# yashsoni501/PQP-for-MPC

Measured on AMD Instinct MI355X. Metric: PQP iterations/sec (and QP-instances/sec) at fixed n_dual, higher is better.
Workload: dtype f32; 1 GPU; BASELINE configs[3] (N=1) / configs[4] (N=8): synthetic n_dual=1024, M=512, 4096 independent problems per GPU, fixed-iteration updateY2; n_dual=1024, batch_per_gpu=4096, global_batch=4096, iters_per_launch=10, parallelism=problem-sharded x1 (no data-path collective)

## Files before the change

### pqp-for-mpc_amd/csrc/pqp_halfsched.h

```cpp
#pragma once

#if defined(__HIPCC__) || defined(__CUDACC__)
#define PQP_HS_HD __host__ __device__ inline
#else
#define PQP_HS_HD inline
#endif

namespace pqp {
namespace hs {

constexpr int kWaves = 16;
constexpr int kTile = 64;
constexpr int kTileStride = 65;
constexpr int kTileWords = kTile * kTileStride;
constexpr int kSlots = 9;
constexpr int kHalfCols = 32;

PQP_HS_HD int steps(int C) { return C > 0 ? kWaves * C + kWaves - 1 : 0; }

PQP_HS_HD int partner(int T, int wave) { return (((T - wave) % kWaves) + kWaves) % kWaves; }

PQP_HS_HD bool active(int T, int wave, int C) {
    const int s = T - wave;
    return s >= 0 && s < kWaves * C;
}
PQP_HS_HD int update_of(int T, int wave) { return (T - wave) / kWaves; }
PQP_HS_HD int kblock_of(int T, int wave) { return (T - wave) % kWaves; }


PQP_HS_HD int tile_rows(int T, int wave) {
    const int p = partner(T, wave);
    return wave < p ? wave : p;
}
PQP_HS_HD int tile_cols(int T, int wave) {
    const int p = partner(T, wave);
    return wave < p ? p : wave;
}
PQP_HS_HD bool transposed(int T, int wave) { return wave > partner(T, wave); }
PQP_HS_HD bool diagonal(int T, int wave) { return partner(T, wave) == wave; }

PQP_HS_HD int load_halves(int T, int wave, int C) {
    if (!active(T, wave, C)) return 0;
    const int p = partner(T, wave);
    return p == wave ? 3 : (wave < p ? 1 : 2);
}

PQP_HS_HD int first_half_col(int halves) { return (halves & 1) ? 0 : kHalfCols; }

PQP_HS_HD int slot(int T, int wave) {
    const int t = ((T % kWaves) + kWaves) % kWaves;
    const int p = partner(T, wave);
    const int lo = wave < p ? wave : p;
    return (wave + p == t) ? lo : lo - (t + 1) / 2;
}

PQP_HS_HD int y_read_buf(int h) { return h & 1; }
PQP_HS_HD int y_write_buf(int h) { return (h + 1) & 1; }

PQP_HS_HD bool last_kblock(int T, int wave) { return kblock_of(T, wave) == kWaves - 1; }

constexpr int kFlagWords = 2 * kSlots + 2 * kWaves;
PQP_HS_HD int tile_flag(int T, int wave, int half) { return 2 * slot(T, wave) + half; }
PQP_HS_HD int y_flag(int buf, int kblock) { return 2 * kSlots + buf * kWaves + kblock; }
PQP_HS_HD int half_of(int halves) { return halves >> 1; }
PQP_HS_HD bool y_dirty(unsigned bits) { return !(bits < 0x7f800000u); }
PQP_HS_HD float q_fold(float s, float q) { return __builtin_fmaf(q, 0.0f, s); }
PQP_HS_HD bool q_dirty(float s) { return s != s; }

}
}
```

### pqp-for-mpc_amd/csrc/pqp_kernels.hip

```cpp
#include <atomic>
#include <type_traits>

#include "pqp_device.h"
#include "pqp_halfsched.h"
#include "pqp_launch.h"

namespace pqp {

static inline unsigned cdiv(long long a, long long b) { return (unsigned)((a + b - 1) / b); }
static bool aligned16(const void* p);

__device__ __forceinline__ float4 ld4(const float* p) { return *reinterpret_cast<const float4*>(p); }
typedef float f32x4 __attribute__((ext_vector_type(4)));
template <bool NTL>
__device__ __forceinline__ float4 ldq4(const float* p) {
    if constexpr (NTL) {
        const f32x4 v = __builtin_nontemporal_load(reinterpret_cast<const f32x4*>(p));
        return make_float4(v.x, v.y, v.z, v.w);
    } else {
        return *reinterpret_cast<const float4*>(p);
    }
}

struct Acc4 {
// ... 50 lines not shown
}

template <bool NTL>
__device__ __forceinline__ void literal_segment(Acc4& a, const float* __restrict__ col, int ldq, int ka, int kb,
                                                const float* __restrict__ y, int row, const float th[4]) {
    int k = ka;
    const float* src = col + (size_t)k * ldq;
    for (; k + 4 <= kb; k += 4) {
        float4 q[4];
#pragma unroll
        for (int j = 0; j < 4; ++j) q[j] = ldq4<NTL>(src + (size_t)j * ldq);
        src += (size_t)4 * ldq;
        const float4 y0 = *reinterpret_cast<const float4*>(y + k);
        literal4(a, q[0], y0.x, k + 0, row, th);
        literal4(a, q[1], y0.y, k + 1, row, th);
        literal4(a, q[2], y0.z, k + 2, row, th);
        literal4(a, q[3], y0.w, k + 3, row, th);
    }
    for (; k < kb; ++k) {
        literal4(a, ldq4<NTL>(src), y[k], k, row, th);
        src += ldq;
    }
}

template <int U, bool NTL, typename OutPtr>
__device__ __forceinline__ void update_rows4(const float* __restrict__ Q, int ldq, int N, int row, int w0,
                                             const float* __restrict__ th_g, const float* __restrict__ fd_g,
                                             const float* __restrict__ y, OutPtr out) {
    Acc4 a;
#pragma unroll
    for (int r = 0; r < 4; ++r) a.p[r] = a.n[r] = 0.0f;
    float th[4];
#pragma unroll
    for (int r = 0; r < 4; ++r) th[r] = (row + r < N) ? th_g[row + r] : 0.0f;
    const float* col = Q + row;
    const int wa = w0 < N ? w0 : N;
    const int wb = (w0 + 256) < N ? (w0 + 256) : N;
    lean_segment<U, NTL>(a, col, ldq, 0, wa, y);
    literal_segment<NTL>(a, col, ldq, wa, wb, y, row, th);
    lean_segment<U, NTL>(a, col, ldq, wb, N, y);
#pragma unroll
    for (int r = 0; r < 4; ++r) {
        const int i = row + r;
        if (i < N) {
            const float f = fd_g[i];
            const float num = a.n[r] + 1.0f * max_ref(0.0f, -f);
            const float den = a.p[r] + 1.0f * max_ref(0.0f, f);
            out[i] = num / den * y[i];
        }
    }
}

template <int NT, int U = 8, bool NTL = false>
__global__ void __launch_bounds__(NT) k_batch_iterate(const float* __restrict__ QdT, long long qstride, int ldq,
                                                      int N, const float* __restrict__ theta,
                                                      const float* __restrict__ Fd, int ldv,
                                                      const float* Y0, float* Y, int updates) {
    extern __shared__ __attribute__((aligned(16))) float lds[];
    float* ya = lds;
    float* yb = lds + ldq;
    const int b = blockIdx.x;
    const int tid = threadIdx.x;
    const float* Q = QdT + (size_t)b * (size_t)qstride;
    const float* th = theta + (size_t)b * ldv;
    const float* fd = Fd + (size_t)b * ldv;
    for (int i = tid; i < ldq; i += NT) {
        ya[i] = (i < N) ? (Y0 ? Y0[(size_t)b * ldv + i] : 1000.0f) : 0.0f;
        yb[i] = 0.0f;
    }
    __syncthreads();
    const int wave = tid >> 6;
    for (int u = 0; u < updates; ++u) {
        float* cur = (u & 1) ? yb : ya;
        float* nxt = (u & 1) ? ya : yb;
        for (int r0 = 0; r0 < N; r0 += 4 * NT) {
            const int row = r0 + 4 * tid;
            const int w0 = r0 + 256 * wave;
            if (row < N) update_rows4<U, NTL, float*>(Q, ldq, N, row, w0, th, fd, cur, nxt);
        }
        __syncthreads();
    }
    const float* fin = (updates & 1) ? yb : ya;
    for (int i = tid; i < N; i += NT) Y[(size_t)b * ldv + i] = fin[i];
}

template <int U, bool NTL>
__device__ __forceinline__ void stream_load(float4 (&q)[U], const float* __restrict__ src, int ldq) {
#pragma unroll
    for (int j = 0; j < U; ++j) q[j] = ldq4<NTL>(src + (size_t)j * ldq);
}
template <int U>
__device__ __forceinline__ void stream_block(Acc4& a, const float4 (&q)[U], int k0, bool literal,
                                             const float* __restrict__ y, int row, const float th[4]) {
    if (literal) {
#pragma unroll
        for (int j = 0; j < U; j += 4) {
            const float4 yv = *reinterpret_cast<const float4*>(y + k0 + j);
            literal4(a, q[j + 0], yv.x, k0 + j + 0, row, th);
            literal4(a, q[j + 1], yv.y, k0 + j + 1, row, th);
            literal4(a, q[j + 2], yv.z, k0 + j + 2, row, th);
            literal4(a, q[j + 3], yv.w, k0 + j + 3, row, th);
        }
    } else {
#pragma unroll
        for (int j = 0; j < U; j += 4) {
            const float4 yv = *reinterpret_cast<const float4*>(y + k0 + j);
            lean4(a, q[j + 0], yv.x);
            lean4(a, q[j + 1], yv.y);
            lean4(a, q[j + 2], yv.z);
            lean4(a, q[j + 3], yv.w);
        }
    }
}
template <int U, bool NTL>
__global__ void __launch_bounds__(256) k_batch_stream(const float* __restrict__ QdT, long long qstride, int ldq,
                                                      int N, const float* __restrict__ theta,
                                                      const float* __restrict__ Fd, int ldv,
                                                      const float* Y0, float* Y, int updates) {
    extern __shared__ __attribute__((aligned(16))) float lds[];
    float* ya = lds;
    float* yb = lds + ldq;
    const int b = blockIdx.x;
    const int tid = threadIdx.x, wave = tid >> 6;
    const float* Q = QdT + (size_t)b * (size_t)qstride;
    const float* th_g = theta + (size_t)b * ldv;
    const float* fd_g = Fd + (size_t)b * ldv;
    for (int i = tid; i < ldq; i += 256) {
        ya[i] = (i < N) ? (Y0 ? Y0[(size_t)b * ldv + i] : 1000.0f) : 0.0f;
        yb[i] = 0.0f;
    }
    const int nb = N / U, npass = N / 1024;
    float4 qa[U], qb[U];
    if (updates > 0) stream_load<U, NTL>(qa, Q + 4 * tid, ldq);
    __syncthreads();
    for (int u = 0; u < updates; ++u) {
        const float* cur = (u & 1) ? yb : ya;
        float* nxt = (u & 1) ? ya : yb;
        for (int pass = 0; pass < npass; ++pass) {
            const int row = pass * 1024 + 4 * tid;
            const int wa = pass * 1024 + 256 * wave, wbd = wa + 256;
            Acc4 a;
#pragma unroll
            for (int r = 0; r < 4; ++r) a.p[r] = a.n[r] = 0.0f;
            float th[4];
#pragma unroll
            for (int r = 0; r < 4; ++r) th[r] = th_g[row + r];
            const float* col = Q + row;
            for (int kb = 0; kb < nb; kb += 2) {
                stream_load<U, NTL>(qb, col + (size_t)(kb + 1) * U * ldq, ldq);
                int k0 = kb * U;
                stream_block<U>(a, qa, k0, k0 >= wa && k0 < wbd, cur, row, th);
                if (kb + 2 < nb) stream_load<U, NTL>(qa, col + (size_t)(kb + 2) * U * ldq, ldq);
                else if (pass + 1 < npass) stream_load<U, NTL>(qa, Q + (pass + 1) * 1024 + 4 * tid, ldq);
                else if (u + 1 < updates) stream_load<U, NTL>(qa, Q + 4 * tid, ldq);
                k0 += U;
                stream_block<U>(a, qb, k0, k0 >= wa && k0 < wbd, cur, row, th);
            }
#pragma unroll
            for (int r = 0; r < 4; ++r) {
                const int i = row + r;
                const float f = fd_g[i];
                const float num = a.n[r] + 1.0f * max_ref(0.0f, -f);
                const float den = a.p[r] + 1.0f * max_ref(0.0f, f);
                nxt[i] = num / den * cur[i];
            }
        }
        __syncthreads();
    }
    const float* fin = (updates & 1) ? yb : ya;
    for (int i = tid; i < N; i += 256) Y[(size_t)b * ldv + i] = fin[i];
}

template <int U, int RL, int RA = 0>
__global__ void __launch_bounds__(256) k_batch_resident(const float* __restrict__ QdT, long long qstride, int ldq,
                                                        const float* __restrict__ theta,
                                                        const float* __restrict__ Fd, int ldv, const float* Y0,
                                                        float* Y, int updates) {
    constexpr int N = 1024, nb = N / U, P = RA + RL;
    static_assert((nb - P) % 2 == 0, "the streamed blocks come in pairs");
    extern __shared__ __attribute__((aligned(16))) float lds[];
    float* ya = lds;
    float* yb = lds + ldq;
    float4* res = reinterpret_cast<float4*>(lds + 2 * ldq);
    const int b = blockIdx.x;
    const int tid = threadIdx.x, wave = tid >> 6;
    const float* Q = QdT + (size_t)b * (size_t)qstride;
    const float* th_g = theta + (size_t)b * ldv;
    const float* fd_g = Fd + (size_t)b * ldv;
    for (int i = tid; i < ldq; i += 256) {
        ya[i] = (i < N) ? (Y0 ? Y0[(size_t)b * ldv + i] : 1000.0f) : 0.0f;
        yb[i] = 0.0f;
    }
    const int row = 4 * tid;
    const int wa = 256 * wave, wbd = wa + 256;
    const float* col = Q + row;
    float th[4];
#pragma unroll
    for (int r = 0; r < 4; ++r) th[r] = th_g[row + r];
    const unsigned long long qaddr = (unsigned long long)Q;
    const __amdgpu_buffer_rsrc_t rs = __builtin_amdgcn_make_buffer_rsrc(
        (void*)(((unsigned long long)__builtin_amdgcn_readfirstlane((unsigned)(qaddr >> 32)) << 32) |
                (unsigned)__builtin_amdgcn_readfirstlane((unsigned)qaddr)),
        (short)0, __builtin_amdgcn_readfirstlane((int)(qstride * 4)), 0x00020000);
    auto ld = [&](float4(&q)[U], int kb, bool nt) {
        if constexpr (RA > 0) {
            const int s0 = kb * U * ldq * 4;
            if (nt) {
#pragma unroll
                for (int j = 0; j < U; ++j) {
                    const f32x4 v = __builtin_amdgcn_raw_buffer_load_b128(rs, 16 * tid, s0 + j * ldq * 4, 2);
                    q[j] = make_float4(v.x, v.y, v.z, v.w);
                }
            } else {
#pragma unroll
                for (int j = 0; j < U; ++j) {
                    const f32x4 v = __builtin_amdgcn_raw_buffer_load_b128(rs, 16 * tid, s0 + j * ldq * 4, 0);
                    q[j] = make_float4(v.x, v.y, v.z, v.w);
                }
            }
        } else {
            if (nt) stream_load<U, true>(q, col + (size_t)kb * U * ldq, ldq);
            else stream_load<U, false>(q, col + (size_t)kb * U * ldq, ldq);
        }
    };
    float4 qa[U], qb[U];
    float4 rr[RA > 0 ? RA * U : 1];
    if (updates > 0) {
#pragma unroll
        for (int rb = 0; rb < RA; ++rb) {
            float4 t[U];
            ld(t, rb, true);
#pragma unroll
            for (int j = 0; j < U; ++j) rr[rb * U + j] = t[j];
        }
        ld(qa, P, false);
    }
    __syncthreads();
    for (int u = 0; u < updates; ++u) {
        const float* cur = (u & 1) ? yb : ya;
        float* nxt = (u & 1) ? ya : yb;
#pragma unroll
        for (int j = 0; j < RA * U; ++j) {
            asm volatile("" : "+a"(rr[j].x));
            asm volatile("" : "+a"(rr[j].y));
            asm volatile("" : "+a"(rr[j].z));
            asm volatile("" : "+a"(rr[j].w));
        }
        Acc4 a;
#pragma unroll
        for (int r = 0; r < 4; ++r) a.p[r] = a.n[r] = 0.0f;
#pragma unroll
        for (int rb = 0; rb < RA; ++rb) {
            float4 q[U];
#pragma unroll
            for (int j = 0; j < U; ++j) q[j] = rr[rb * U + j];
            const int k0 = rb * U;
            stream_block<U>(a, q, k0, k0 >= wa && k0 < wbd, cur, row, th);
        }
#pragma unroll
        for (int lb = 0; lb < RL; ++lb) {
            float4* slot = res + (size_t)lb * U * 256 + tid;
            if (u == 0) {
                ld(qb, RA + lb, true);
#pragma unroll
                for (int j = 0; j < U; ++j) slot[j * 256] = qb[j];
            } else {
#pragma unroll
                for (int j = 0; j < U; ++j) qb[j] = slot[j * 256];
            }
            const int k0 = (RA + lb) * U;
            stream_block<U>(a, qb, k0, k0 >= wa && k0 < wbd, cur, row, th);
        }
        for (int kb = P; kb < nb; kb += 2) {
            ld(qb, kb + 1, true);
            int k0 = kb * U;
            stream_block<U>(a, qa, k0, k0 >= wa && k0 < wbd, cur, row, th);
            if (kb + 2 < nb)
                ld(qa, kb + 2, true);
            else if (u + 1 < updates)
                ld(qa, P, false);
            k0 += U;
            stream_block<U>(a, qb, k0, k0 >= wa && k0 < wbd, cur, row, th);
        }
#pragma unroll
        for (int r = 0; r < 4; ++r) {
            const int i = row + r;
            const float f = fd_g[i];
            const float num = a.n[r] + 1.0f * max_ref(0.0f, -f);
            const float den = a.p[r] + 1.0f * max_ref(0.0f, f);
            nxt[i] = num / den * cur[i];
        }
        __syncthreads();
    }
    const float* fin = (updates & 1) ? yb : ya;
    for (int i = tid; i < N; i += 256) Y[(size_t)b * ldv + i] = fin[i];
}

__device__ __forceinline__ void lean1(float& ap, float& an, float q, float y) {
    const float z = 0.0f * y;
    const float p = q * y;
    ap += (q < 0.0f) ? z : p;
    an += (q > 0.0f) ? z : -p;
}
template <int SK, bool DIAG>
__device__ __forceinline__ void half_tile_sum(float& ap, float& an, const float* __restrict__ q,
                                              const float* __restrict__ yk, int lane, float th) {
    constexpr int CH = 8;
#pragma unroll 1
    for (int c = 0; c < hs::kTile; c += CH) {
        float qv[CH];
#pragma unroll
        for (int j = 0; j < CH; ++j) qv[j] = q[(c + j) * SK];
#pragma unroll
        for (int j = 0; j < CH; j += 4) {
            const float4 yv = *reinterpret_cast<const float4*>(yk + c + j);
            if constexpr (DIAG) {
                literal1(ap, an, qv[j + 0], yv.x, (c + j + 0 == lane) ? th : 0.0f);
                literal1(ap, an, qv[j + 1], yv.y, (c + j + 1 == lane) ? th : 0.0f);
                literal1(ap, an, qv[j + 2], yv.z, (c + j + 2 == lane) ? th : 0.0f);
                literal1(ap, an, qv[j + 3], yv.w, (c + j + 3 == lane) ? th : 0.0f);
            } else {
                lean1(ap, an, qv[j + 0], yv.x);
                lean1(ap, an, qv[j + 1], yv.y);
                lean1(ap, an, qv[j + 2], yv.z);
                lean1(ap, an, qv[j + 3], yv.w);
            }
        }
    }
}
typedef float hf2 __attribute__((ext_vector_type(2)));
template <int SK>
__device__ __forceinline__ void half_tile_sum_pf(float& ap, float& an, const float* __restrict__ q,
                                                 const float* __restrict__ yk) {
    constexpr int CH = 16;
    hf2 acc = {ap, an};
#pragma unroll 1
    for (int c = 0; c < hs::kTile; c += CH) {
        float qv[CH];
#pragma unroll
        for (int j = 0; j < CH; ++j) qv[j] = q[(c + j) * SK];
#pragma unroll
        for (int j = 0; j < CH; j += 4) {
            const float4 yv = *reinterpret_cast<const float4*>(yk + c + j);
            const hf2 p01 = hf2{qv[j + 0], qv[j + 1]} * hf2{yv.x, yv.y};
            const hf2 p23 = hf2{qv[j + 2], qv[j + 3]} * hf2{yv.z, yv.w};
#pragma unroll
            for (int h = 0; h < 4; ++h) {
                const float p = h < 2 ? p01[h] : p23[h - 2];
                float tp, tn;
                asm("v_max_f32 %0, %1, 0" : "=v"(tp) : "v"(p));
                asm("v_max_f32_e64 %0, -%1, 0" : "=v"(tn) : "v"(p));
                acc += hf2{tp, tn};
            }
        }
    }
    ap = acc.x;
    an = acc.y;
}
__device__ __forceinline__ int half_y_flag(float y) {
    return __builtin_amdgcn_ballot_w64(hs::y_dirty(__float_as_uint(y))) != 0;
}
__device__ __forceinline__ float half_q_fold(float s, f32x4 q) {
    return hs::q_fold(hs::q_fold(hs::q_fold(hs::q_fold(s, q.x), q.y), q.z), q.w);
}
constexpr size_t kHalfLdsBytes =
    ((size_t)2 * 1024 + (size_t)hs::kSlots * hs::kTileWords + hs::kFlagWords) * sizeof(float);
static_assert(kHalfLdsBytes <= 160 * 1024, "k_batch_half: LDS of a gfx950 CU");
template <bool PF>
__global__ void __launch_bounds__(1024) k_batch_half(const float* __restrict__ QdT, long long qstride, int ldq,
                                                     const float* __restrict__ theta, const float* __restrict__ Fd,
                                                     int ldv, const float* Y0, float* Y, int updates) {
    constexpr int N = 1024;
    constexpr int HL = hs::kHalfCols / 4;
    extern __shared__ __attribute__((aligned(16))) float lds[];
    float* ybuf = lds;
    float* tiles = lds + 2 * N;
    int* flags = reinterpret_cast<int*>(tiles + hs::kSlots * hs::kTileWords);
    const int b = blockIdx.x;
    const int tid = threadIdx.x, lane = tid & 63;
    const int wave = __builtin_amdgcn_readfirstlane(tid >> 6);
    const float* Q = QdT + (size_t)b * (size_t)qstride;
    const int row = hs::kTile * wave + lane;
    const float ys = Y0 ? Y0[(size_t)b * ldv + tid] : 1000.0f;
    ybuf[tid] = ys;
    ybuf[N + tid] = 0.0f;
    if constexpr (PF) {
        flags[hs::y_flag(0, wave)] = half_y_flag(ys);
        flags[hs::y_flag(1, wave)] = 1;
    }
    const float th = theta[(size_t)b * ldv + row];
    const float f = Fd[(size_t)b * ldv + row];
    const int lk = lane >> 4, lr = 4 * (lane & 15);
    f32x4 pa[HL], pb[HL];
    auto issue = [&](int T) {
        const int halves = hs::load_halves(T, wave, updates);
        if (halves == 0) return;
        const int k0 = hs::kTile * hs::tile_cols(T, wave) + hs::first_half_col(halves) + lk;
        const float* src = Q + (size_t)k0 * ldq + hs::kTile * hs::tile_rows(T, wave) + lr;
#pragma unroll
        for (int j = 0; j < HL; ++j)
            pa[j] = __builtin_nontemporal_load(reinterpret_cast<const f32x4*>(src + (size_t)(4 * j) * ldq));
        if (halves == 3) {
#pragma unroll
            for (int j = 0; j < HL; ++j)
                pb[j] = __builtin_nontemporal_load(
                    reinterpret_cast<const f32x4*>(src + (size_t)(hs::kHalfCols + 4 * j) * ldq));
        }
    };
    auto stash = [&](int T) {
        const int halves = hs::load_halves(T, wave, updates);
        if (halves == 0) return;
        float* dst = tiles + hs::slot(T, wave) * hs::kTileWords + (hs::first_half_col(halves) + lk) * hs::kTileStride + lr;
        float fold = 0.0f;
#pragma unroll
        for (int j = 0; j < HL; ++j) {
            float* d = dst + 4 * j * hs::kTileStride;
            d[0] = pa[j].x, d[1] = pa[j].y, d[2] = pa[j].z, d[3] = pa[j].w;
            if constexpr (PF) fold = half_q_fold(fold, pa[j]);
        }
        if constexpr (PF) {
            if (halves != 3)
                flags[hs::tile_flag(T, wave, hs::half_of(halves))] =
                    __builtin_amdgcn_ballot_w64(hs::q_dirty(fold)) != 0;
        }
        if (halves == 3) {
#pragma unroll
            for (int j = 0; j < HL; ++j) {
                float* d = dst + (hs::kHalfCols + 4 * j) * hs::kTileStride;
                d[0] = pb[j].x, d[1] = pb[j].y, d[2] = pb[j].z, d[3] = pb[j].w;
            }
        }
    };
    const int S = hs::steps(updates);
    issue(0);
    __syncthreads();
    if (updates == 0) Y[(size_t)b * ldv + tid] = ybuf[tid];
    float ap = 0.0f, an = 0.0f;
    for (int T = 0; T < S; ++T) {
        stash(T);
        __syncthreads();
        issue(T + 1);
        if (hs::active(T, wave, updates)) {
            const int h = hs::update_of(T, wave), K = hs::kblock_of(T, wave);
            const float* cur = ybuf + hs::y_read_buf(h) * N;
            const float* yk = cur + hs::kTile * K;
            const float* tile = tiles + hs::slot(T, wave) * hs::kTileWords;
            if (K == 0) ap = an = 0.0f;
            if (hs::diagonal(T, wave))
                half_tile_sum<hs::kTileStride, true>(ap, an, tile + lane, yk, lane, th);
            else {
                bool fast = false;
                if constexpr (PF) {
                    const int dirty = flags[hs::tile_flag(T, wave, 0)] | flags[hs::tile_flag(T, wave, 1)] |
                                      flags[hs::y_flag(hs::y_read_buf(h), K)];
                    fast = __builtin_amdgcn_readfirstlane(dirty) == 0;
                }
                if (hs::transposed(T, wave)) {
                    if (fast) half_tile_sum_pf<1>(ap, an, tile + lane * hs::kTileStride, yk);
                    else half_tile_sum<1, false>(ap, an, tile + lane * hs::kTileStride, yk, lane, th);
                } else {
                    if (fast) half_tile_sum_pf<hs::kTileStride>(ap, an, tile + lane, yk);
                    else half_tile_sum<hs::kTileStride, false>(ap, an, tile + lane, yk, lane, th);
                }
            }
            if (hs::last_kblock(T, wave)) {
                const float num = an + 1.0f * max_ref(0.0f, -f);
                const float den = ap + 1.0f * max_ref(0.0f, f);
                const float yn = num / den * cur[row];
                ybuf[hs::y_write_buf(h) * N + row] = yn;
                if constexpr (PF)
                    flags[hs::y_flag(hs::y_write_buf(h), wave)] = half_y_flag(yn);
                if (h == updates - 1) Y[(size_t)b * ldv + row] = yn;
            }
        }
        __syncthreads();
    }
}

template <int NT, int U = 8, bool NTL = false>
__global__ void __launch_bounds__(NT) k_batch_update(const float* __restrict__ QdT, long long qstride, int ldq,
                                                     int N, const float* __restrict__ theta,
                                                     const float* __restrict__ Fd, int ldv,
                                                     const float* __restrict__ Yin, float* __restrict__ Yout) {
    extern __shared__ __attribute__((aligned(16))) float lds[];
    const int b = blockIdx.y;
    const int tid = threadIdx.x;
    const float* yg = Yin + (size_t)b * ldv;
    for (int i = tid; i < ldq; i += NT) lds[i] = (i < N) ? yg[i] : 0.0f;
    __syncthreads();
    const int r0 = blockIdx.x * 4 * NT;
    const int row = r0 + 4 * tid;
    const int w0 = r0 + 256 * (tid >> 6);
    if (row < N)
        update_rows4<U, NTL>(QdT + (size_t)b * (size_t)qstride, ldq, N, row, w0, theta + (size_t)b * ldv,
                     Fd + (size_t)b * ldv, lds, Yout + (size_t)b * ldv);
}

__global__ void __launch_bounds__(256) k_update_split(const float* __restrict__ QpT, const float* __restrict__ QnT,
                                                      int ldq, int N, const float* __restrict__ Fdp,
                                                      const float* __restrict__ Fdn, const float* __restrict__ Y,
                                                      float* __restrict__ Ynext) {
    const int i = blockIdx.x * 256 + threadIdx.x;
    if (i >= N) return;
    float num = 0.0f, den = 0.0f;
    for (int k = 0; k < N; ++k) num += QnT[(size_t)k * ldq + i] * Y[k];
    for (int k = 0; k < N; ++k) den += QpT[(size_t)k * ldq + i] * Y[k];
    num = num + 1.0f * Fdn[i];
    den = den + 1.0f * Fdp[i];
    Ynext[i] = num / den * Y[i];
}

__host__ __device__ inline int split_wgs(int rows, int lw) { return (2 * rows + lw - 1) / lw; }

__global__ void __launch_bounds__(256) k_build_split(const float* __restrict__ Qd, int ld,
                                                     const float* __restrict__ theta, const float* __restrict__ Fd,
                                                     int N, int rows, int row0, int lw, float* __restrict__ SP,
                                                     float* __restrict__ fdpn) {
    const int KB = split_kblocks(N);
    const long long e = (long long)blockIdx.x * 256 + threadIdx.x;
    if (e < (long long)rows * 4 * KB) {
        const int i = (int)(e / (4 * KB)), k = (int)(e % (4 * KB));
        float qn = 0.0f, qp = 0.0f;
        if (k < N) {
            const float q = Qd[(size_t)i * ld + k];
            const float t = (row0 + i == k) ? theta[i] : 0.0f;
            qn = max_ref(0.0f, -q) + 1.0f * t;
            qp = max_ref(0.0f, q) + 1.0f * t;
        }
        const int p = 2 * i;
        const size_t base = (((size_t)(p / lw) * KB + (k >> 2)) * lw + (p % lw)) * 4 + (k & 3);
        SP[base] = qn;
        SP[base + 4] = qp;
    }
    if (e < rows) {
        const float fd = Fd[row0 + e];
        fdpn[2 * e + 0] = max_ref(0.0f, -fd);
        fdpn[2 * e + 1] = max_ref(0.0f, fd);
    }
}

__global__ void __launch_bounds__(256) k_theta_rows(const float* __restrict__ Qd, int ld, int N, int rows,
                                                    float* __restrict__ theta) {
    const int i = blockIdx.x * 256 + threadIdx.x;
    if (i >= rows) return;
    float s = 0.0f;
    for (int k = 0; k < N; ++k) s += max_ref(0.0f, -Qd[(size_t)i * ld + k]) * 1.0f;
    theta[i] = max_ref(s, 5.0f);
}

__device__ inline void stage_y_lds(const float* __restrict__ Y, int N, int n_lds, float* ys) {
    const int t = threadIdx.x;
    int done = 0;
    if ((reinterpret_cast<uintptr_t>(Y) & 15) == 0) {
        const int N4 = N >> 2;
        const float4* Y4 = reinterpret_cast<const float4*>(Y);
        for (int b = 0; b < N4; b += 64 * 8) {
            float4 v[8];
#pragma unroll
            for (int j = 0; j < 8; ++j) {
                const int i = b + 64 * j + t;
                v[j] = (i < N4) ? Y4[i] : make_float4(0.0f, 0.0f, 0.0f, 0.0f);
            }
#pragma unroll
            for (int j = 0; j < 8; ++j) {
                const int i = b + 64 * j + t;
                if (i < N4) reinterpret_cast<float4*>(ys)[i] = v[j];
            }
        }
        done = 4 * N4;
    }
    for (int b = done; b < n_lds; b += 64 * 16) {
        float v[16];
#pragma unroll
        for (int j = 0; j < 16; ++j) {
            const int k = b + 64 * j + t;
            v[j] = (k < N) ? Y[k] : 0.0f;
        }
#pragma unroll
        for (int j = 0; j < 16; ++j) {
            const int k = b + 64 * j + t;
            if (k < n_lds) ys[k] = v[j];
        }
    }
    __syncthreads();
}

template <int W, int S>
__global__ void __launch_bounds__(64 * W) k_split_relay(const float* __restrict__ SP, const float* __restrict__ fdpn,
                                                        int N, int rows, int row0, int lw,
                                                        const float* __restrict__ Yin, float* __restrict__ Yout,
                                                        const int* __restrict__ gate, int* __restrict__ err,
                                                        int spin_max) {
    if (gate && *gate != kStatusContinue) return;
    extern __shared__ __attribute__((aligned(16))) float lds[];
    unsigned long long* slot = reinterpret_cast<unsigned long long*>(lds);
    float* ys = lds + 128;
    const int KB = split_kblocks(N);
    const int lane = threadIdx.x & 63, w = __builtin_amdgcn_readfirstlane(threadIdx.x >> 6);
    const int ll = lane % lw;
    const int p = blockIdx.x * lw + ll;
    const bool live = lane < lw && p < 2 * rows;
    const int G = (KB + S - 1) / S;
    typedef float f4v __attribute__((ext_vector_type(4)));
    typedef float f2v __attribute__((ext_vector_type(2)));
    const float* region = SP + (size_t)blockIdx.x * KB * lw * 4;
    const __amdgpu_buffer_rsrc_t rs =
        __builtin_amdgcn_make_buffer_rsrc(const_cast<float*>(region), (short)0, KB * lw * 16, 0x00020000);
    const int vo = ll * 16, kstride = lw * 16;
    f4v q[S];
    const bool lane_loads = lane < lw;
    auto load_seg = [&](int g) {
        const int nj = KB - g * S;
#pragma unroll
        for (int j = 0; j < S; ++j)
            q[j] = (j < nj && lane_loads) ? __builtin_amdgcn_raw_buffer_load_b128(rs, vo, (g * S + j) * kstride, 0)
                                          : f4v{0.0f, 0.0f, 0.0f, 0.0f};
    };
    if (w < G) load_seg(w);
    const float fd = live ? fdpn[p] : 0.0f;
    {
        const int t = threadIdx.x, n_lds = 4 * G * S;
        for (int b = 0; b < n_lds; b += 64 * W * 8) {
            float v[8];
#pragma unroll
            for (int j = 0; j < 8; ++j) {
                const int k = b + 64 * W * j + t;
                v[j] = (k < N) ? Yin[k] : 0.0f;
            }
#pragma unroll
            for (int j = 0; j < 8; ++j) {
                const int k = b + 64 * W * j + t;
                if (k < n_lds) ys[k] = v[j];
            }
        }
        if (w == 0) slot[lane] = 0ull;
    }
    __syncthreads();
    float acc = 0.0f;
    bool stale = false;
    for (int g = w; g < G; g += W) {
#pragma unroll
        for (int j0 = 0; j0 < S; j0 += 4) {
            f4v y[4];
#pragma unroll
            for (int u = 0; u < 4; ++u) y[u] = *reinterpret_cast<const f4v*>(ys + 4 * (g * S + j0 + u));
#pragma unroll
            for (int u = 0; u < 4; ++u) {
                const int j = j0 + u;
                const f2v lo = f2v{q[j].x, q[j].y} * f2v{y[u].x, y[u].y};
                const f2v hi = f2v{q[j].z, q[j].w} * f2v{y[u].z, y[u].w};
                q[j] = f4v{lo.x, lo.y, hi.x, hi.y};
            }
#pragma unroll
            for (int u = 0; u < 4; ++u) asm volatile("" : "+v"(q[j0 + u]));
        }
        const unsigned long long h = relay_wait(slot, lane, g, spin_max, stale);
        __builtin_amdgcn_s_setprio(3);
        acc = __uint_as_float((unsigned)h);
#pragma unroll
        for (int j = 0; j < S; ++j) {
            acc += q[j].x;
            acc += q[j].y;
            acc += q[j].z;
            acc += q[j].w;
        }
        __hip_atomic_store(slot + lane, ((unsigned long long)(g + 1) << 32) | __float_as_uint(acc), __ATOMIC_RELAXED,
                           __HIP_MEMORY_SCOPE_WORKGROUP);
        __builtin_amdgcn_s_setprio(0);
        if (g + W < G) load_seg(g + W);
    }
    if (w == (G - 1) % W) {
        const float v = acc + 1.0f * fd;
        const float den = __shfl_xor(v, 1);
        if (!(p & 1) && live) {
            const int i = p >> 1;
            Yout[i] = v / den * ys[row0 + i];
        }
    }
    relay_report(stale, err, lane);
}

constexpr int kLeanS = 16;
__global__ void __launch_bounds__(256) k_build_lean(const float* __restrict__ Qd, int ld,
                                                    const float* __restrict__ theta, const float* __restrict__ Fd,
                                                    int N, int rows, int row0, int lw, float* __restrict__ LP,
                                                    float* __restrict__ aux) {
    const int KB = split_kblocks(N);
    const int rp = lw >> 1;
    const long long e = (long long)blockIdx.x * 256 + threadIdx.x;
    if (e < (long long)rows * 4 * KB) {
        const int i = (int)(e / (4 * KB)), k = (int)(e % (4 * KB));
        const size_t at = (((size_t)(i / rp) * KB + (k >> 2)) * rp + (i % rp)) * 4 + (k & 3);
        const float q = k < N ? Qd[(size_t)i * ld + k] : 0.0f;
        LP[at] = q;
        if (q != q) {
            const int G = (KB + kLeanS - 1) / kLeanS, nwg = (rows + rp - 1) / rp;
            int* segnan = reinterpret_cast<int*>(aux + 4 * (size_t)nwg * rp);
            atomicOr(segnan + (size_t)(i / rp) * G + (k >> 2) / kLeanS, 1);
        }
    }
    if (e < rows) {
        const float fd = Fd[row0 + e];
        aux[4 * e + 0] = max_ref(0.0f, -fd);
        aux[4 * e + 1] = max_ref(0.0f, fd);
        aux[4 * e + 2] = theta[e];
        aux[4 * e + 3] = 0.0f;
    }
}

template <int W, int S>
__global__ void __launch_bounds__(64 * W) k_lean_relay(const float* __restrict__ LP, const float* __restrict__ aux,
                                                       int N, int rows, int row0, int lw,
                                                       const float* __restrict__ Yin, float* __restrict__ Yout,
                                                       const int* __restrict__ gate, int* __restrict__ err,
                                                       int spin_max) {
    if (gate && *gate != kStatusContinue) return;
    extern __shared__ __attribute__((aligned(16))) float lds[];
    unsigned long long* slot = reinterpret_cast<unsigned long long*>(lds);
    float* ys = lds + 128;
    const int KB = split_kblocks(N);
    const int lane = threadIdx.x & 63, w = __builtin_amdgcn_readfirstlane(threadIdx.x >> 6);
    const int ll = lane % lw;
    const int rp = lw >> 1;
    const int side = ll & 1;
    const int r = blockIdx.x * rp + (ll >> 1);
    const bool live = lane < lw && r < rows;
    const int G = (KB + S - 1) / S;
    typedef float f4v __attribute__((ext_vector_type(4)));
    const float* region = LP + (size_t)blockIdx.x * KB * rp * 4;
    const __amdgpu_buffer_rsrc_t rs =
        __builtin_amdgcn_make_buffer_rsrc(const_cast<float*>(region), (short)0, KB * rp * 16, 0x00020000);
    const int vo = (ll >> 1) * 16, kstride = rp * 16;
// ... 4217 lines not shown
```

Measured before the change: 2.726 million instance-iterations/s.

## Exploit diagonal tile symmetry and pack LDS tile stores as float2

Diagonal tiles now fetch only one half plus the missing lower-right quadrant from global memory, then fill the remaining quadrant by mirroring the already-loaded half in LDS. This relies on the tile being symmetric. The LDS tile stride changes from 65 to 66 so stores and reads can use 8-byte float2 accesses instead of scalar ones. This cuts global traffic on diagonal tiles and the LDS instruction count, but the padding change may reintroduce bank conflicts and slightly raises LDS use.

```diff
diff --git a/pqp-for-mpc_amd/csrc/pqp_halfsched.h b/pqp-for-mpc_amd/csrc/pqp_halfsched.h
--- a/pqp-for-mpc_amd/csrc/pqp_halfsched.h
+++ b/pqp-for-mpc_amd/csrc/pqp_halfsched.h
@@ -11,7 +11,7 @@
 
 constexpr int kWaves = 16;
 constexpr int kTile = 64;
-constexpr int kTileStride = 65;
+constexpr int kTileStride = 66;
 constexpr int kTileWords = kTile * kTileStride;
 constexpr int kSlots = 9;
 constexpr int kHalfCols = 32;
@@ -47,6 +47,16 @@
 
 PQP_HS_HD int first_half_col(int halves) { return (halves & 1) ? 0 : kHalfCols; }
 
+constexpr int kPieceRows = 4;
+constexpr int kHalfLoads = 8;
+constexpr int kQuadLoads = 4;
+PQP_HS_HD int tile_word(int i, int k) { return k * kTileStride + i; }
+PQP_HS_HD int piece_row(int lane) { return kPieceRows * ((lane & 7) | ((lane >> 1) & 8)); }
+PQP_HS_HD int piece_col(int lane) { return ((lane >> 3) & 1) | ((lane >> 4) & 2); }
+PQP_HS_HD int quad_row(int lane) { return kHalfCols + kPieceRows * (lane & 7); }
+PQP_HS_HD int quad_col(int lane) { return kHalfCols + (lane >> 3); }
+PQP_HS_HD bool mirrors(int lane) { return piece_row(lane) >= kHalfCols; }
+
 PQP_HS_HD int slot(int T, int wave) {
     const int t = ((T % kWaves) + kWaves) % kWaves;
     const int p = partner(T, wave);
diff --git a/pqp-for-mpc_amd/csrc/pqp_kernels.hip b/pqp-for-mpc_amd/csrc/pqp_kernels.hip
--- a/pqp-for-mpc_amd/csrc/pqp_kernels.hip
+++ b/pqp-for-mpc_amd/csrc/pqp_kernels.hip
@@ -376,6 +376,21 @@
     ap += (q < 0.0f) ? z : p;
     an += (q > 0.0f) ? z : -p;
 }
+typedef float hf2 __attribute__((ext_vector_type(2)));
+typedef volatile hf2 __attribute__((address_space(3))) lds_hf2;
+template <int SK, int CH>
+__device__ __forceinline__ void half_tile_entries(float (&qv)[CH], const float* __restrict__ q) {
+    if constexpr (SK == 1) {
+#pragma unroll
+        for (int j = 0; j < CH; j += 2) {
+            const hf2 v = *(const lds_hf2*)(q + j);
+            qv[j] = v.x, qv[j + 1] = v.y;
+        }
+    } else {
+#pragma unroll
+        for (int j = 0; j < CH; ++j) qv[j] = q[j * SK];
+    }
+}
 template <int SK, bool DIAG>
 __device__ __forceinline__ void half_tile_sum(float& ap, float& an, const float* __restrict__ q,
                                               const float* __restrict__ yk, int lane, float th) {
@@ -383,8 +398,7 @@
 #pragma unroll 1
     for (int c = 0; c < hs::kTile; c += CH) {
         float qv[CH];
-#pragma unroll
-        for (int j = 0; j < CH; ++j) qv[j] = q[(c + j) * SK];
+        half_tile_entries<SK, CH>(qv, q + c * SK);
 #pragma unroll
         for (int j = 0; j < CH; j += 4) {
             const float4 yv = *reinterpret_cast<const float4*>(yk + c + j);
@@ -402,7 +416,6 @@
         }
     }
 }
-typedef float hf2 __attribute__((ext_vector_type(2)));
 template <int SK>
 __device__ __forceinline__ void half_tile_sum_pf(float& ap, float& an, const float* __restrict__ q,
                                                  const float* __restrict__ yk) {
@@ -411,8 +424,7 @@
 #pragma unroll 1
     for (int c = 0; c < hs::kTile; c += CH) {
         float qv[CH];
-#pragma unroll
-        for (int j = 0; j < CH; ++j) qv[j] = q[(c + j) * SK];
+        half_tile_entries<SK, CH>(qv, q + c * SK);
 #pragma unroll
         for (int j = 0; j < CH; j += 4) {
             const float4 yv = *reinterpret_cast<const float4*>(yk + c + j);
@@ -436,6 +448,10 @@
 }
 __device__ __forceinline__ float half_q_fold(float s, f32x4 q) {
     return hs::q_fold(hs::q_fold(hs::q_fold(hs::q_fold(s, q.x), q.y), q.z), q.w);
+}
+__device__ __forceinline__ void half_store_piece(float* d, f32x4 v) {
+    *(lds_hf2*)d = hf2{v.x, v.y};
+    *(lds_hf2*)(d + 2) = hf2{v.z, v.w};
 }
 constexpr size_t kHalfLdsBytes =
     ((size_t)2 * 1024 + (size_t)hs::kSlots * hs::kTileWords + hs::kFlagWords) * sizeof(float);
@@ -445,7 +461,7 @@
                                                      const float* __restrict__ theta, const float* __restrict__ Fd,
                                                      int ldv, const float* Y0, float* Y, int updates) {
     constexpr int N = 1024;
-    constexpr int HL = hs::kHalfCols / 4;
+    constexpr int HL = hs::kHalfLoads, QL = hs::kQuadLoads;
     extern __shared__ __attribute__((aligned(16))) float lds[];
     float* ybuf = lds;
     float* tiles = lds + 2 * N;
@@ -464,32 +480,33 @@
     }
     const float th = theta[(size_t)b * ldv + row];
     const float f = Fd[(size_t)b * ldv + row];
-    const int lk = lane >> 4, lr = 4 * (lane & 15);
-    f32x4 pa[HL], pb[HL];
+    const int lk = hs::piece_col(lane), lr = hs::piece_row(lane);
+    const int qk = hs::quad_col(lane), qr = hs::quad_row(lane);
+    f32x4 pa[HL], pb[QL];
     auto issue = [&](int T) {
         const int halves = hs::load_halves(T, wave, updates);
         if (halves == 0) return;
-        const int k0 = hs::kTile * hs::tile_cols(T, wave) + hs::first_half_col(halves) + lk;
-        const float* src = Q + (size_t)k0 * ldq + hs::kTile * hs::tile_rows(T, wave) + lr;
+        const float* tile0 = Q + (size_t)(hs::kTile * hs::tile_cols(T, wave)) * ldq + hs::kTile * hs::tile_rows(T, wave);
+        const float* src = tile0 + (size_t)(hs::first_half_col(halves) + lk) * ldq + lr;
 #pragma unroll
         for (int j = 0; j < HL; ++j)
             pa[j] = __builtin_nontemporal_load(reinterpret_cast<const f32x4*>(src + (size_t)(4 * j) * ldq));
         if (halves == 3) {
-#pragma unroll
-            for (int j = 0; j < HL; ++j)
-                pb[j] = __builtin_nontemporal_load(
-                    reinterpret_cast<const f32x4*>(src + (size_t)(hs::kHalfCols + 4 * j) * ldq));
+            const float* qsrc = tile0 + (size_t)qk * ldq + qr;
+#pragma unroll
+            for (int j = 0; j < QL; ++j)
+                pb[j] = __builtin_nontemporal_load(reinterpret_cast<const f32x4*>(qsrc + (size_t)(8 * j) * ldq));
         }
     };
     auto stash = [&](int T) {
         const int halves = hs::load_halves(T, wave, updates);
         if (halves == 0) return;
-        float* dst = tiles + hs::slot(T, wave) * hs::kTileWords + (hs::first_half_col(halves) + lk) * hs::kTileStride + lr;
+        float* tile = tiles + hs::slot(T, wave) * hs::kTileWords;
+        float* dst = tile + hs::tile_word(lr, hs::first_half_col(halves) + lk);
         float fold = 0.0f;
 #pragma unroll
         for (int j = 0; j < HL; ++j) {
-            float* d = dst + 4 * j * hs::kTileStride;
-            d[0] = pa[j].x, d[1] = pa[j].y, d[2] = pa[j].z, d[3] = pa[j].w;
+            half_store_piece(dst + 4 * j * hs::kTileStride, pa[j]);
             if constexpr (PF) fold = half_q_fold(fold, pa[j]);
         }
         if constexpr (PF) {
@@ -498,10 +515,17 @@
                     __builtin_amdgcn_ballot_w64(hs::q_dirty(fold)) != 0;
         }
         if (halves == 3) {
-#pragma unroll
-            for (int j = 0; j < HL; ++j) {
-                float* d = dst + (hs::kHalfCols + 4 * j) * hs::kTileStride;
-                d[0] = pb[j].x, d[1] = pb[j].y, d[2] = pb[j].z, d[3] = pb[j].w;
+            float* qdst = tile + hs::tile_word(qr, qk);
+#pragma unroll
+            for (int j = 0; j < QL; ++j) half_store_piece(qdst + 8 * j * hs::kTileStride, pb[j]);
+            if (hs::mirrors(lane)) {
+                float* mdst = tile + hs::tile_word(lk, lr);
+#pragma unroll
+                for (int j = 0; j < HL; ++j) {
+                    float* d = mdst + 4 * j;
+                    d[0] = pa[j].x, d[hs::kTileStride] = pa[j].y, d[2 * hs::kTileStride] = pa[j].z,
+                    d[3 * hs::kTileStride] = pa[j].w;
+                }
             }
         }
     };
```

New measurement: 2.942 million instance-iterations/s, median of 6. +7.9%, better.
